# scraed/LanPaint

Measured on AMD Instinct MI355X. Metric: langevin_think_iterations_per_sec, higher is better.
Workload: dtype f32; 1 GPU; c2_sdxl: latent 1x4x128x128 per GPU, 30 sigmas x 5 think iterations, 50% box mask, stub backbone x->(0.9x,0.8x), VE/Karras schedule; rng=torch, graph=auto, mask_format=f32, mask_seen_by_kernels=bits, captured_calls=1, backbone_io=f32, replicas=1, rows_per_gpu=1, global_rows=1, latent_elements_per_gpu=65536

## Files before the change

### __graft_entry__.py

```python
from __future__ import annotations

import os
import subprocess
import sys

ROOT = os.path.dirname(os.path.abspath(__file__))
if ROOT not in sys.path:
    sys.path.insert(0, ROOT)


def build() -> None:
    from lanpaint_amd import build as lp_build
    lp_build.build(force=False, verbose=True)
    subprocess.run(["make", "-s", "-C", os.path.join(ROOT, "oracle")], check=True)
    import lanpaint_amd
    from lanpaint_amd import _cabi
    lib = _cabi.load()
    assert lib.lp_abi_version() == _cabi.ABI_VERSION
    print("lanpaint_amd", lanpaint_amd.__version__, "->", _cabi.LIB_PATH)


def smoke() -> None:
    import numpy as np
    import torch
    from lanpaint_amd import LanPaint
    from oracle.lanpaint_oracle import OracleLanPaint, times_from_sigma
    from tests.stubs import LinearTupleModel

    assert torch.cuda.is_available(), "smoke() needs a HIP device"
    dev = torch.device("cuda", 0)
    rng = np.random.default_rng(0)
    shape = (1, 4, 16, 16)
    y = rng.standard_normal(shape, dtype=np.float32)
    noise = rng.standard_normal(shape, dtype=np.float32)
    sigma = np.float32([1.5])
    x = (y + noise * sigma[0]).astype(np.float32)
    mask = np.zeros(shape, dtype=np.float32)
    mask[..., :8] = 1.0
    times = times_from_sigma(sigma, False)
    draws = [rng.standard_normal(shape, dtype=np.float32) for _ in range(5)]

    it = iter(draws)
# ... 42 lines not shown
```

### lanpaint_amd/build.py

```python
from __future__ import annotations

import os
import shutil
import subprocess
import sys

HERE = os.path.dirname(os.path.abspath(__file__))
ROOT = os.path.dirname(HERE)
CSRC = os.path.join(HERE, "csrc")
SOURCES = ["step_kernel.hip", "aux_kernels.hip", "blend_kernel.hip", "videomask_kernel.hip", "audio_kernel.hip",
           "detail_kernel.hip", "label_kernel.hip", "color_kernel.hip", "fill_kernel.hip",
           "multiband_kernel.hip", "refine_kernel.hip", "stabilize_kernel.hip", "grain_kernel.hip",
           "propagate_kernel.hip", "temporal_fill_kernel.hip", "temporal_smooth_kernel.hip",
           "shot_kernel.hip", "cabi.hip"]
HEADERS = [os.path.join(CSRC, "lp_common.h"), os.path.join(CSRC, "mask_tile.h"), os.path.join(CSRC, "resample_tile.h"),
           os.path.join(CSRC, "motion_tile.h"), os.path.join(CSRC, "exports.map"), os.path.join(ROOT, "include", "lanpaint_hip.h")]
OUT = os.path.join(HERE, "liblanpaint_hip.so")


def _hipcc():
    for cand in (os.environ.get("HIPCC"), shutil.which("hipcc"), "/opt/rocm/bin/hipcc"):
        if cand and os.path.exists(cand):
            return cand
    raise RuntimeError("hipcc not found (set HIPCC or install ROCm)")


def needs_build(out=OUT):
    if not os.path.exists(out):
        return True
    t = os.path.getmtime(out)
    deps = [os.path.join(CSRC, s) for s in SOURCES] + HEADERS
    return any(os.path.getmtime(p) > t for p in deps)


def build(force=False, verbose=True, shader_clock=False, trace=False):
    if trace:
        out = os.path.join(ROOT, "build", "liblanpaint_hip_trace.so")
        os.makedirs(os.path.dirname(out), exist_ok=True)
        return _compile(out, ["-DLP_TRACE_INSTANTIATIONS"], verbose) if force or needs_build(out) else out
    if shader_clock:
        out = os.path.join(ROOT, "build", "liblanpaint_hip_clk.so")
        os.makedirs(os.path.dirname(out), exist_ok=True)
        return _compile(out, ["-DLP_SHADER_CLOCK"], verbose) if force or needs_build(out) else out
    if not force and not needs_build():
        return OUT
    return _compile(OUT, [], verbose)


def _compile(out, extra, verbose):
    cmd = [_hipcc(), "--offload-arch=gfx950", "-O3", "-std=c++17", "-ffp-contract=on", "-fno-fast-math",
           "-fhip-fp32-correctly-rounded-divide-sqrt", "-fPIC", "-shared", "-fvisibility=hidden",
           "-Wl,--version-script=" + os.path.join(CSRC, "exports.map"),
           "-mllvm", "-amdgpu-kernarg-preload-count=14",
           "-I" + os.path.join(ROOT, "include"), "-I" + CSRC]
    cmd += extra + [os.path.join(CSRC, s) for s in SOURCES] + ["-o", out]
    if verbose:
        print(" ".join(cmd), flush=True)
    subprocess.run(cmd, check=True)
    return out


if __name__ == "__main__":
    build(force="--force" in sys.argv, shader_clock="--shader-clock" in sys.argv, trace="--trace" in sys.argv)
```

### lanpaint_amd/capture.py

```python
from __future__ import annotations

import ctypes
import os
import weakref

import torch

from . import _cabi
from ._util import _gc_hold, _gc_release
from .buffers import _CapturedCall, _Workspace
from .masks import _compact_mask


class GraphReplay:

    MAX_GRAPHS = 16
    AUTO_MAX_BACKBONE_HOST_US = 100.0

    def begin_call(self, x, latent_image, noise, sigma, latent_mask, current_times, model_options, seed):
        cap = self._last_cap
        if cap is None or cap.tail is None or self.model_dtype is not None or not x.is_cuda:
            return None
        self.img_dim_size = len(x.shape)
        self.latent_image, self.noise = latent_image, noise
        self.audio_indicator = self.current_times_audio = self.audio_correction = None
        self._noise_regenerated = self._noise_is_zero(noise)
        if not self._same_call(cap, x, sigma, latent_mask, current_times, cap.ident[4], model_options, seed):
            return None
        lib, stream = self._lib, self._stream(x.device)
        ve, abt = current_times[0], current_times[1]
        out = torch.empty_like(x)
        k0 = cap.k0_desc
# ... 45 lines not shown
        if table is None or table[3] != len(self._graphs) or table[4] is not model_options:
            nd.valid_word = self._rng_state(x.device).data_ptr() + 32
            table = self._node_table(cap0, nd.n_steps, model_options, nd)
        stream = self._stream(x.device)
        ve, abt = current_times[0], current_times[1]
        out = torch.empty_like(x)
        k0 = cap0.k0_desc
        k0.x, k0.noise = x.data_ptr(), noise.data_ptr()
        k0.t_ve, k0.t_abt, k0.t_rsig = ve.data_ptr(), abt.data_ptr(), sigma.data_ptr()
        k0.t_model = (current_times[2] if cap0.flow else ve).data_ptr()
        k0.io_table_val[0], k0.io_table_val[1] = k0.x, out.data_ptr()
        off = 0
        if self.rng == "torch":
            gen = self._generator(x.device)
            off = gen.get_offset()
            k0.rng_state_val[0], k0.rng_state_val[1] = off, gen.initial_seed()
        if getattr(nd, "_lp_table", None) is not table:
            nd._lp_table = table
            nd.replace, nd.exec_by_count, nd.n_counts = table[2], table[0], len(table[1])
            nd.valid_word = self._rng_state(x.device).data_ptr() + 32
            nd.full_exec_by_count, nd.full_binding_by_count = table[5], table[6]
        rc = self._lib.lp_node_call(ctypes.byref(nd), stream)
        if rc != _cabi.LP_OK:
            try:
                self._rng_state(x.device)[4] = 1
            except Exception:
                pass
            self._forget_captures()
            _cabi.check(rc, "lp_node_call")
        n_eff = nd.n_eff
        if not nd.launched:
            cap0.node_table = None
            return self(x, latent_image, noise, sigma, latent_mask, current_times, model_options, seed, n_steps=n_eff), n_eff
        cap = table[1][n_eff]
        if self.rng == "torch" and cap.launches:
            self._generator(x.device).set_offset(off + cap.launches)
            self._torch_consumed += cap.launches
        self._iterations_run += cap.ran
        self.last_inner_steps = cap.ran
        return out, n_eff

    def _forget_captures(self):
        self._last_cap = None
        for cap in self._graphs.values():
            cap.alive = False
            cap.node_table = None
            cap.siblings = {}
        self._graphs.clear()

    def _node_table(self, cap0, n_max, model_options, nd=None):
        caps = []
        for n in range(int(n_max) + 1):
            cap = cap0 if cap0.ident[4] == n else cap0.siblings.get(n)
            if cap is None or not cap.alive:
                cap = self._graphs.get(cap0.key[:2] + (n,) + cap0.key[3:])
                if cap is not None and (cap.tail is None or cap.model_options is not model_options or cap.ws is not cap0.ws):
                    cap = None
                if cap is not None:
                    cap0.siblings[n] = cap
            caps.append(cap if (cap is not None and cap.tail is not None) else None)
        arr = (ctypes.c_void_p * len(caps))(*[(c.tail.graph_exec if c is not None else None) for c in caps])
        full = full_b = None
        if nd is not None and os.environ.get("LANPAINT_AMD_NODE_ONE_LAUNCH", "1") != "0":
# ... 407 lines not shown
```

### lanpaint_amd/csrc/cabi.hip

```cpp
#include <cmath>

#include "lp_common.h"

namespace lp {
int step_dispatch(const lp_step_desc* d, hipStream_t stream, void* timer);
int replace_node_update(const lp_step_desc* d, hipGraphExec_t exec, const lp_graph_binding* b);
int timer_create(void** out);
int timer_destroy(void* h);
int timer_elapsed_ns(void* h, double* ns);
int coeffs_dispatch(const lp_hyper* h, const float* ve, int ve_stride, const float* abt, int abt_stride,
                    const float* rs, int rs_stride, const float* step_ov, int step_stride, const float* t_model,
                    int t_stride, int rows, float* table, hipStream_t stream);
int finalize_dispatch(const lp_final_desc* d, hipStream_t stream);
int sigma_times_dispatch(const float* sigma, int rows, const float* schedule, int schedule_len, int is_flow, float* times,
                         float* scalars, int32_t* seq_out, int32_t seq, hipStream_t stream);
int sigma_times_rule_dispatch(const float* sigma, int rows, const float* schedule, int schedule_len, int is_flow,
                              float* times, float* scalars, int32_t* seq_out, int32_t seq, int32_t n_steps, int32_t early_stop,
                              int32_t total_steps, double min_step_frac, int32_t guess, uint64_t* valid_out, hipStream_t stream);
int blend_dispatch(const lp_blend_desc* d, hipStream_t stream);
int philox_dispatch(float* out, int64_t n_el, uint64_t seed, uint64_t offset, uint32_t slot, hipStream_t stream);
int ring_dispatch(const float* mask, float* ring, int64_t planes, int height, int width, hipStream_t stream);
int wmse_dispatch(const float* a, const float* b, const float* mask, const float* ring, int64_t n_el, double* acc,
                  double* scratch, int scratch_blocks, hipStream_t stream);
int torch_normal_dispatch(float* out, int64_t n, uint64_t seed, uint64_t offset, uint32_t bg, hipStream_t stream);
// ... 400 lines not shown
int lp_graph_release(void* tail_graph, void* tail_exec) {
    if (tail_exec) (void)hipGraphExecDestroy(static_cast<hipGraphExec_t>(tail_exec));
    if (tail_graph) (void)hipGraphDestroy(static_cast<hipGraph_t>(tail_graph));
    return LP_OK;
}

int32_t lp_effective_inner_steps(int32_t n_steps, double step_f, double frac, int32_t total_steps, int32_t early_stop,
                                 double min_step_frac) {
    return lp::effective_inner_steps(n_steps, step_f, frac, total_steps, early_stop, min_step_frac);
}

static int node_wait(const lp_node_call_desc* c, int32_t want, hipStream_t s) {
    for (int32_t k = 0; k < c->spin_limit; ++k)
        if (__atomic_load_n(c->seq_out, __ATOMIC_ACQUIRE) == want) return LP_OK;
    if (hipStreamSynchronize(s) != hipSuccess) return LP_E_LAUNCH;
    return __atomic_load_n(c->seq_out, __ATOMIC_ACQUIRE) == want ? LP_OK : LP_E_LAUNCH;
}

static int node_call_body(lp_node_call_desc* c, hipStream_t s, bool* queued_spec) {
    const auto exec_for = [&](int32_t n) -> hipGraphExec_t {
        return (c->exec_by_count && n >= 0 && n < c->n_counts) ? static_cast<hipGraphExec_t>(c->exec_by_count[n]) : nullptr;
    };
    const bool speculate = c->guess >= 0 && c->valid_word && exec_for(c->guess) != nullptr && c->replace && !c->replace->es_reset;
    c->speculated = speculate ? 1 : 0;
    c->hit = 0;
    c->launched = 0;
    int rc = LP_OK;
    lp_step_desc rep;
    if (c->replace) {
        rep = *c->replace;
        rep.io_valid = 0;
    }
    lp_step_desc d;
    bool fold_sigma = speculate && c->fold_sigma && c->is_flow == ((c->replace->flags & LP_FL_FLOW) ? 1 : 0) &&
                      c->rows == c->replace->rows;
    if (fold_sigma) {
        d = rep;
        d.phases |= LP_PH_SIGMA;
        d.sg_sigma = c->sigma; d.sg_schedule = c->schedule; d.sg_schedule_len = c->schedule_len; d.sg_times_out = c->times_out;
        d.sg_scalars_out = c->scalars_out; d.sg_seq_out = c->seq_out; d.sg_seq = c->seq; d.sg_valid_out = c->valid_word;
        d.sg_n_steps = c->n_steps; d.sg_early_stop = c->early_stop; d.sg_total_steps = c->total_steps; d.sg_guess = c->guess;
        d.sg_min_step_frac = c->min_step_frac;
        lp::StepPlan plan;
        fold_sigma = lp::plan_step(d, &plan) == LP_OK;
    }
    c->one_launch = 0;
    if (fold_sigma) {
        hipGraphExec_t full = (c->full_exec_by_count && c->full_binding_by_count && c->guess < c->n_counts)
                                  ? static_cast<hipGraphExec_t>(c->full_exec_by_count[c->guess]) : nullptr;
        const lp_graph_binding* fb = full ? c->full_binding_by_count[c->guess] : nullptr;
        if (full && fb) {
            rc = lp::replace_node_update(&d, full, fb);
            if (rc != LP_OK) return rc;
            if (hipGraphLaunch(full, s) != hipSuccess) return LP_E_LAUNCH;
            *queued_spec = true;
            c->one_launch = 1;
        } else {
            rc = lp::step_dispatch(&d, s, nullptr);
            if (rc != LP_OK) return rc;
            *queued_spec = true;
        }
    } else {
        rc = lp::sigma_times_rule_dispatch(c->sigma, c->rows, c->schedule, c->schedule_len, c->is_flow, c->times_out,
                                           c->scalars_out, c->seq_out, c->seq, c->n_steps, c->early_stop, c->total_steps,
                                           c->min_step_frac, speculate ? c->guess : -1, c->valid_word, s);
        if (rc != LP_OK) return rc;
        *queued_spec = speculate;
        if (c->replace) {
            rc = lp::step_dispatch(&rep, s, nullptr);
            if (rc != LP_OK) return rc;
        }
    }
    if (speculate && !c->one_launch && hipGraphLaunch(exec_for(c->guess), s) != hipSuccess) return LP_E_LAUNCH;
    rc = node_wait(c, c->seq, s);
    if (rc != LP_OK) return rc;
    c->step_f = c->scalars_out[0];
    c->frac = c->scalars_out[1];
    c->n_eff = lp::effective_inner_steps(c->n_steps, static_cast<double>(c->step_f), static_cast<double>(c->frac),
                                         c->total_steps, c->early_stop, c->min_step_frac);
    if (c->valid_word && static_cast<int32_t>(c->scalars_out[3]) != c->n_eff) return LP_E_UNSUPPORTED;
    if (speculate) {
        if (c->n_eff == c->guess) {
            c->hit = 1;
            c->launched = 1;
// ... 84 lines not shown
```

### lanpaint_amd/csrc/lp_common.h

```cpp
#pragma once
#include <hip/hip_runtime.h>
#include <hip/hip_ext.h>
#include <stdint.h>

#include "lanpaint_hip.h"

namespace lp {

constexpr int kWave = 64;

__device__ __forceinline__ int nearest_exact_index(int i, int in_size, int out_size, int rule) {
#pragma clang fp contract(off)
    const float scale = static_cast<float>(in_size) / static_cast<float>(out_size);
    const float at = static_cast<float>(i) + 0.5f;
    int s;
    if (rule == LP_NN_ATEN_SCALAR) {
        s = static_cast<int>(floorf(at * scale));
    } else {
        float src = (rule == LP_NN_ATEN_CPU_GENERIC_FMA) ? __builtin_fmaf(scale, at, -0.5f) : (scale * at - 0.5f);
        src = src < 0.0f ? 0.0f : src;
        s = static_cast<int>(floorf(static_cast<float>(static_cast<double>(src) + 0.5)));
    }
    return s < in_size - 1 ? s : in_size - 1;
}
// ... 583 lines not shown
}

struct StepPlan {
    const void* kernel;
    dim3 grid;
    uint32_t ph_ct;
    int vec;
    bool decide;
    int decide_slot;
    int mode, x0w, rng, es;
    bool st;
};
struct StepArgs {
    void* x_t;
    void* C;
    const void *a2, *a3, *a4, *a5;
    int32_t el_per_row;
    uint32_t flags;
    void* ptr[9];
};
int plan_step(const lp_step_desc& d, StepPlan* out, bool timed = false);
void pack_step_args(const StepPlan& p, const lp_step_desc& d, StepArgs* a);
bool plan_is_node(const StepPlan& p, const void* func, const dim3& grid, const dim3& block);

__device__ __forceinline__ int code_of(float v) {
    const float t = v > 0.0f ? (v < 1.0f ? v : 1.0f) : 0.0f;
    return static_cast<int>(__fadd_rn(__fmul_rn(t, 255.0f), 0.5f));
}

__device__ __forceinline__ double capped_distance(int32_t q) {
    const uint32_t mag = q < 0 ? 0u - static_cast<uint32_t>(q) : static_cast<uint32_t>(q);
    const double r = sqrt(static_cast<double>(mag < 4096u ? mag : 4096u));
    return q < 0 ? -r : r;
}

}
```

### lanpaint_amd/csrc/step_kernel.hip

```cpp
#include <cstddef>

#include "lp_common.h"

#pragma clang fp contract(off)

namespace lp {

struct RegionCoef {
    float e_full, k_full, std_full, e_half, k_half, std_half, dt, a, cx0, cxt;
};

struct RowCoef {
    float scale, sqrt_abt, oma, abt, rsigma, dtx, dty, ax, ay, dx, dy, valid;
    RegionCoef reg[2];
    float rscale;
};

__device__ __forceinline__ RowCoef load_row(const float* __restrict__ coef, int row) {
    const float* c = coef + static_cast<int64_t>(row) * LP_COEF_STRIDE;
    RowCoef r;
    r.scale = c[LP_C_SCALE]; r.sqrt_abt = c[LP_C_SQRT_ABT]; r.oma = c[LP_C_OMA]; r.abt = c[LP_C_ABT];
    r.rsigma = c[LP_C_RSIGMA]; r.dtx = c[LP_C_DTX]; r.dty = c[LP_C_DTY]; r.ax = c[LP_C_AX]; r.ay = c[LP_C_AY];
    r.dx = c[LP_C_DX]; r.dy = c[LP_C_DY]; r.valid = c[LP_C_VALID];
    r.rscale = c[LP_C_RSCALE];
// ... 1482 lines not shown
static int enqueue(const StepPlan& p, const lp_step_desc& d, hipStream_t stream, Timer* timer) {
    LP_TRACE(p);
    StepArgs a;
    pack_step_args(p, d, &a);
    if (timer) (void)hipExtLaunchKernel(p.kernel, p.grid, dim3(kBlock), a.ptr, 0, stream, timer->start, timer->stop, 0);
    else (void)hipLaunchKernel(p.kernel, p.grid, dim3(kBlock), a.ptr, 0, stream);
    if (hipGetLastError() != hipSuccess) return LP_E_LAUNCH;
    if (p.decide) {
        hipLaunchKernelGGL(lp_es_decide_kernel, dim3(1), dim3(kWave), 0, stream, d, p.decide_slot);
        if (hipGetLastError() != hipSuccess) return LP_E_LAUNCH;
    }
    return LP_OK;
}

int step_dispatch(const lp_step_desc* dp, hipStream_t stream, void* timer_handle) {
    if (!dp) return LP_E_INVALID;
    Timer* timer = static_cast<Timer*>(timer_handle);
    StepPlan p;
    const int rc = plan_step(*dp, &p, timer != nullptr);
    return rc == LP_OK ? enqueue(p, *dp, stream, timer) : rc;
}

int replace_node_update(const lp_step_desc* dp, hipGraphExec_t exec, const lp_graph_binding* b) {
    if (!dp || !exec || !b || !b->node || !b->func) return LP_E_INVALID;
    const lp_step_desc& d = *dp;
    if (!(d.phases & LP_PH_REPLACE) || d.xi_post || d.xi_pre || (d.flags & LP_FL_X0S_GIVEN)) return LP_E_INVALID;
    StepPlan p;
    const int rc = plan_step(d, &p);
    if (rc != LP_OK) return rc;
    if (!plan_is_node(p, b->func, dim3(b->grid[0], b->grid[1], b->grid[2]), dim3(b->block[0], b->block[1], b->block[2])))
        return LP_E_INVALID;
    StepArgs a;
    pack_step_args(p, d, &a);
    hipKernelNodeParams np{};
    np.func = const_cast<void*>(p.kernel);
    np.gridDim = p.grid;
    np.blockDim = dim3(kBlock);
    np.sharedMemBytes = b->shared_bytes;
    np.kernelParams = a.ptr;
    np.extra = nullptr;
    return hipGraphExecKernelNodeSetParams(exec, static_cast<hipGraphNode_t>(b->node), &np) == hipSuccess ? LP_OK : LP_E_LAUNCH;
}

int timer_create(void** out) {
    if (!out) return LP_E_INVALID;
    Timer* t = new Timer();
    if (hipEventCreate(&t->start) != hipSuccess || hipEventCreate(&t->stop) != hipSuccess) {
        delete t;
        return LP_E_LAUNCH;
    }
    *out = t;
    return LP_OK;
// ... 23 lines not shown
```

### lanpaint_amd/nodes.py

```python
from __future__ import annotations

import math
import os
import weakref
from contextlib import contextmanager

import torch

from . import _cabi, interp_rule
from .blend import MaskBlend, gaussian_kernel_2d, merge_video_with_mask
from .image_nodes import LanPaint_ImageDecode, LanPaint_ImageEncode, _snap_mask_nearest_exact
from .resample import _hip_device, _resample
from .lanpaint import LanPaint, pack_mask, raw_stream, refresh_packed_mask, tensor_version
from .types import FusedCFGHeads

try:
    import comfy
    import comfy.samplers
    from comfy.model_base import ModelType
    HAVE_COMFY = True
except Exception:
    comfy = None
    HAVE_COMFY = False

    class ModelType:
        FLUX = "FLUX"
        FLOW = "FLOW"
        FLOW_AV = "FLOW_AV"

try:
    import comfyui_version
    _ver = tuple(int(p) if p.isdigit() else 0 for p in comfyui_version.__version__.split("."))
# ... 162 lines not shown
                                          self.conds.get("positive", None), self.cfg, self.cfg_BIG,
                                          model_options=model_options, seed=seed)


class KSamplerX0Inpaint:

    def __init__(self, model, sigmas):
        self.inner_model = model
        self.sigmas = sigmas
        self.audio_indicator = None
        self.audio_shifts = None
        self._mask_cache = None
        self._mailbox = None
        self._seq = 0
        self._node_desc = None
        self._node_static = None
        self._speculate = os.environ.get("LANPAINT_AMD_SPECULATE", "1") != "0"
        self._last_step = None
        self._spec_misses = 0
        self._spec_hist = []
        self._n_eff_table = None
        self._sched = None
        self._times = None

    def _guess_inner_steps(self, nd, rows, flow):
        if self._last_step is None or self._spec_misses >= 2 or not self._speculate:
            return -1
        tab = self._n_eff_table
        key = (rows, flow, nd.n_steps, nd.early_stop, nd.min_step_frac)
        if tab is None or tab[0] != key:
            import numpy as np
            sched = self._sched[1].detach().cpu().numpy().astype(np.float32)
            one = np.float32(1.0)
            counts = []
            for j, s in enumerate(sched):
                if flow:
                    a = one - s
                    abt = (a * a) / (a * a + s * s) if (a * a + s * s) != 0 else np.float32(np.nan)
                else:
                    abt = one / (one + s * s)
                acc = np.float32(0.0)
                for _ in range(rows):
                    acc = np.float32(acc + np.float32(one - abt))
                frac = float(np.float32(acc / np.float32(rows)))
                counts.append(-1 if frac != frac else
                              _cabi.load().lp_effective_inner_steps(nd.n_steps, float(j), frac, nd.total_steps, nd.early_stop,
                                                                    nd.min_step_frac))
            self._n_eff_table = tab = (key, counts)
        j = self._last_step + 1
        return tab[1][j] if 0 <= j < len(tab[1]) else -1

    def _mailbox_views(self):
        if self._mailbox is None:
            mb = torch.zeros(4, dtype=torch.float32).pin_memory()
            self._mailbox = (mb, mb.numpy(), mb.view(torch.int32).numpy())
        return self._mailbox

    def _wait_mailbox(self, seq, device):
        _mb, f32, i32 = self._mailbox
        for _ in range(20000):
            if i32[2] == seq:
                break
        else:
            torch.cuda.current_stream(device).synchronize()
            if i32[2] != seq:
                raise RuntimeError("lp_sigma_times mailbox was not written (sequence %d, found %d)" % (seq, int(i32[2])))
        return float(f32[0]), float(f32[1])

    def _latent_mask(self, denoise_mask):
        c = self._mask_cache
        ver = (tensor_version(denoise_mask), denoise_mask.data_ptr())
        if (c is not None and c[0]() is denoise_mask and c[1][1] == ver[1] and denoise_mask.is_cuda
                and (c[1][0] != ver[0] or ver[0] == -1) and getattr(c[2], "_lp_bits", None) is not None):
            refresh_packed_mask(c[2], denoise_mask)
            self._mask_cache = c = (c[0], ver, c[2])
            return c[2]
        if c is None or c[0]() is not denoise_mask or c[1] != ver:
            if denoise_mask.is_cuda:
                latent_mask = pack_mask(denoise_mask, denoise_mask=True)
            else:
                latent_mask = 1 - (denoise_mask > 0.5).float()
            self._mask_cache = c = (weakref.ref(denoise_mask), ver, latent_mask)
        return c[2]

    def __call__(self, x, sigma, denoise_mask, model_options={}, seed=None, **kwargs):
        model_type = self.inner_model.inner_model.model_type
        IS_FLUX = model_type == ModelType.FLUX
        IS_FLOW = model_type in FLOW_MODEL_TYPES
        fused_seq = None
        if (sigma.is_cuda and sigma.dtype == torch.float32 and sigma.ndim == 1 and self.sigmas.is_cuda
                and self.sigmas.dtype == torch.float32 and self.sigmas.device == sigma.device):
            sc = self._sched
            if sc is None or sc[0] is not self.sigmas:
                dense = self.sigmas.contiguous()
                self._sched = sc = (self.sigmas, dense, dense.data_ptr(), dense.numel(), len(self.sigmas) - 1)
            sig_c = sigma if sigma.is_contiguous() else sigma.contiguous()
            rows = sig_c.shape[0]
            tm = self._times
            if tm is None or tm[0] != rows or tm[1] != sigma.device:
                sets = []
                for _ in range(2):
                    b = torch.empty((3 * rows,), dtype=torch.float32, device=sigma.device)
                    sets.append((b[:rows], b[rows:2 * rows], b[2 * rows:3 * rows], b))
                self._times = tm = (rows, sigma.device, sets)
            VE_Sigma, abt, Flow_t, buf = tm[2][self._seq & 1]
            mb = self._mailbox_views()[0]
            self._seq = fused_seq = (self._seq % 0x7ffffff0) + 1
            pm = getattr(self, "PaintMethod", None)
            if (denoise_mask is not None and self.audio_indicator is None and "denoise_mask_function" not in model_options
                    and getattr(pm, "_last_cap", None) is not None and sigma.device.index == torch.cuda.current_device()
                    and type(self.LanPaint_early_stop) is int and type(pm.n_steps) is int):
                nd = self._node_desc
                if nd is None:
                    nd = self._node_desc = _cabi.LpNodeCallDesc()
                    nd.spin_limit = 200000
                    nd.fold_sigma = int(os.environ.get("LANPAINT_AMD_FOLD_SIGMA", "1") != "0")
                static = (rows, sc[2], sc[3], bool(IS_FLUX or IS_FLOW), pm.n_steps, self.LanPaint_early_stop, sc[4],
                          getattr(self, "LanPaint_min_step_frac", 1.0), mb)
                if self._node_static != static:
                    self._node_static = static
                    nd.rows, nd.schedule, nd.schedule_len, nd.is_flow = rows, sc[2], sc[3], int(static[3])
                    nd.scalars_out, nd.seq_out = mb.data_ptr(), mb.data_ptr() + 8
                    nd.n_steps, nd.early_stop, nd.total_steps = int(pm.n_steps), int(self.LanPaint_early_stop), sc[4]
                    nd.min_step_frac = float(static[7])
                nd.sigma, nd.seq, nd.times_out = sig_c.data_ptr(), fused_seq, buf.data_ptr()
                nd.guess = self._guess_inner_steps(nd, rows, static[3])
                res = pm.node_call(x, self.latent_image, self.noise, sigma, self._latent_mask(denoise_mask),
                                   (VE_Sigma, abt, Flow_t), model_options, seed, nd)
                if res is not None:
                    out = res[0]
                    self._last_step = int(nd.step_f)
                    if nd.speculated:
                        self._spec_hist = (self._spec_hist + [bool(nd.hit)])[-4:]
                        if self._spec_hist.count(False) >= 2:
                            self._spec_misses = 2
                    step_i = model_options.get("i", kwargs.get("i", 0))
                    if step_i % 2 == 0:
                        cb = model_options.get("callback", None)
                        if cb is not None:
                            cb({"i": step_i, "denoised": out, "x": x})
                    return out
            args = (sig_c.data_ptr(), rows, sc[2], sc[3], int(bool(IS_FLUX or IS_FLOW)), buf.data_ptr(),
                    mb.data_ptr(), mb.data_ptr() + 8, fused_seq, raw_stream(sigma.device))
            if sigma.device.index == torch.cuda.current_device():
                _cabi.check(_cabi.load().lp_sigma_times_mailbox(*args), "lp_sigma_times_mailbox")
            else:
                with torch.cuda.device(sigma.device):
                    _cabi.check(_cabi.load().lp_sigma_times_mailbox(*args), "lp_sigma_times_mailbox")
        elif IS_FLUX or IS_FLOW:
            Flow_t = sigma
            abt = (1 - Flow_t) ** 2 / ((1 - Flow_t) ** 2 + Flow_t ** 2)
            VE_Sigma = Flow_t / (1 - Flow_t)
        else:
            VE_Sigma = sigma
            abt = 1 / (1 + VE_Sigma ** 2)
            Flow_t = (1 - abt) ** 0.5 / ((1 - abt) ** 0.5 + abt ** 0.5)

        current_times_audio = audio_correction = None
        if self.audio_indicator is not None and self.audio_shifts is not None and time_shift_sigma is not None:
            shift_v, shift_a = self.audio_shifts
            Flow_a = time_shift_sigma(Flow_t, shift_v, shift_a)
            abt_a = (1 - Flow_a) ** 2 / ((1 - Flow_a) ** 2 + Flow_a ** 2)
            current_times_audio = (Flow_a / (1 - Flow_a), abt_a, Flow_a)
# ... 387 lines not shown
```

Before: 125,500 think-iterations/s.

## Add native C++ node-call fast path that replays captured graphs without Python

Adds a pybind/torch C++ extension (NodeFast) that snapshots the engine state after a successful captured node call. On later calls it validates a list of watched attributes, tensor pins and versions natively, then calls lp_node_call directly, skipping the Python sampler-facing path. The native node call also reorders descriptor setup so a planned graph update reuses the already computed step plan. This targets per-call host overhead in a workload dominated by small kernels. In exchange it adds a large snapshot/validation surface where stale-state bugs are possible, plus a build dependency that falls back to Python if missing.

```diff
diff --git a/__graft_entry__.py b/__graft_entry__.py
--- a/__graft_entry__.py
+++ b/__graft_entry__.py
@@ -18,6 +18,8 @@
     lib = _cabi.load()
     assert lib.lp_abi_version() == _cabi.ABI_VERSION
     print("lanpaint_amd", lanpaint_amd.__version__, "->", _cabi.LIB_PATH)
+    from lanpaint_amd import nodefast
+    print("native node-call entry:", getattr(nodefast.load(), "__file__", "not built (the Python path is the path)"))
 
 
 def smoke() -> None:
diff --git a/lanpaint_amd/build.py b/lanpaint_amd/build.py
--- a/lanpaint_amd/build.py
+++ b/lanpaint_amd/build.py
@@ -16,6 +16,8 @@
 HEADERS = [os.path.join(CSRC, "lp_common.h"), os.path.join(CSRC, "mask_tile.h"), os.path.join(CSRC, "resample_tile.h"),
            os.path.join(CSRC, "motion_tile.h"), os.path.join(CSRC, "exports.map"), os.path.join(ROOT, "include", "lanpaint_hip.h")]
 OUT = os.path.join(HERE, "liblanpaint_hip.so")
+NODE_FAST_SOURCE = "node_fast.cpp"
+NODE_FAST_OUT = os.path.join(HERE, "_node_fast.so")
 
 
 def _hipcc():
@@ -42,9 +44,40 @@
         out = os.path.join(ROOT, "build", "liblanpaint_hip_clk.so")
         os.makedirs(os.path.dirname(out), exist_ok=True)
         return _compile(out, ["-DLP_SHADER_CLOCK"], verbose) if force or needs_build(out) else out
-    if not force and not needs_build():
-        return OUT
-    return _compile(OUT, [], verbose)
+    out = OUT if (not force and not needs_build()) else _compile(OUT, [], verbose)
+    build_node_fast(force=force, verbose=verbose)
+    return out
+
+
+def build_node_fast(force=False, verbose=True):
+    src, hdr = os.path.join(CSRC, NODE_FAST_SOURCE), os.path.join(ROOT, "include", "lanpaint_hip.h")
+    if not force and os.path.exists(NODE_FAST_OUT) and os.path.getmtime(NODE_FAST_OUT) >= max(os.path.getmtime(src), os.path.getmtime(hdr)):
+        return NODE_FAST_OUT
+    try:
+        import sysconfig
+        import pybind11
+        import torch
+        from torch.utils import cpp_extension
+        cxx = os.environ.get("CXX") or shutil.which("g++") or shutil.which("c++") or shutil.which("clang++")
+        if cxx is None:
+            raise RuntimeError("no C++ compiler found (set CXX)")
+        rocm = os.environ.get("ROCM_PATH") or os.path.dirname(os.path.dirname(os.path.realpath(_hipcc())))
+        incs = cpp_extension.include_paths() + [pybind11.get_include(), sysconfig.get_paths()["include"],
+                                                os.path.join(rocm, "include"), os.path.join(ROOT, "include")]
+        libdir = os.path.join(os.path.dirname(torch.__file__), "lib")
+        cmd = [cxx, "-O2", "-std=c++17", "-fPIC", "-shared", "-fvisibility=hidden", "-D__HIP_PLATFORM_AMD__=1", "-DUSE_ROCM=1",
+               "-D_GLIBCXX_USE_CXX11_ABI=%d" % int(torch._C._GLIBCXX_USE_CXX11_ABI)]
+        cmd += ["-I" + p for p in incs] + [src, "-o", NODE_FAST_OUT, "-L" + libdir, "-Wl,-rpath," + libdir,
+                                           "-lc10", "-lc10_hip", "-ltorch_cpu", "-ltorch", "-ltorch_python"]
+        if verbose:
+            print(" ".join(cmd), flush=True)
+        subprocess.run(cmd, check=True)
+        return NODE_FAST_OUT
+    except Exception as e:
+        import warnings
+        warnings.warn("lanpaint_amd: the native node-call entry was not built (%s: %s); the sampler-facing path stays in Python"
+                      % (type(e).__name__, str(e).splitlines()[0] if str(e) else ""))
+        return None
 
 
 def _compile(out, extra, verbose):
diff --git a/lanpaint_amd/capture.py b/lanpaint_amd/capture.py
--- a/lanpaint_amd/capture.py
+++ b/lanpaint_amd/capture.py
@@ -7,7 +7,7 @@
 import torch
 
 from . import _cabi
-from ._util import _gc_hold, _gc_release
+from ._util import _gc_hold, _gc_release, tensor_version
 from .buffers import _CapturedCall, _Workspace
 from .masks import _compact_mask
 
@@ -99,16 +99,10 @@
             nd.full_exec_by_count, nd.full_binding_by_count = table[5], table[6]
         rc = self._lib.lp_node_call(ctypes.byref(nd), stream)
         if rc != _cabi.LP_OK:
-            try:
-                self._rng_state(x.device)[4] = 1
-            except Exception:
-                pass
-            self._forget_captures()
-            _cabi.check(rc, "lp_node_call")
+            self._node_call_failed(rc, x.device)
         n_eff = nd.n_eff
         if not nd.launched:
-            cap0.node_table = None
-            return self(x, latent_image, noise, sigma, latent_mask, current_times, model_options, seed, n_steps=n_eff), n_eff
+            return self._node_call_uncaptured(x, sigma, latent_mask, current_times, model_options, seed, n_eff), n_eff
         cap = table[1][n_eff]
         if self.rng == "torch" and cap.launches:
             self._generator(x.device).set_offset(off + cap.launches)
@@ -116,6 +110,47 @@
         self._iterations_run += cap.ran
         self.last_inner_steps = cap.ran
         return out, n_eff
+
+    def _node_call_failed(self, rc, dev):
+        try:
+            self._rng_state(dev)[4] = 1
+        except Exception:
+            pass
+        self._forget_captures()
+        _cabi.check(rc, "lp_node_call")
+
+    def _node_call_uncaptured(self, x, sigma, latent_mask, current_times, model_options, seed, n_eff):
+        if self._last_cap is not None:
+            self._last_cap.node_table = None
+        return self(x, self.latent_image, self.noise, sigma, latent_mask, current_times, model_options, seed, n_steps=n_eff)
+
+    def node_fast_state(self, x, sigma, latent_mask, current_times, model_options, seed, nd):
+        cap0 = self._last_cap
+        table = None if cap0 is None else cap0.node_table
+        if (table is None or getattr(nd, "_lp_table", None) is not table or table[3] != len(self._graphs)
+                or table[4] is not model_options or self.rng not in ("torch", "philox") or not isinstance(model_options, dict)
+                or not self._same_call(cap0, x, sigma, latent_mask, current_times, cap0.ident[4], model_options, seed)
+                or (tensor_version(self.noise) == -1 and not self.assume_static_noise)):
+            return None
+        t, own = type(self), ("langevin_dynamics", "score_model", "prepare_step_size", "node_call")
+        if any(n in self.__dict__ for n in own) or not isinstance(self._lib.lp_node_call, ctypes._CFuncPtr):
+            return None
+        ident = lambda o, *names: [(o, n, getattr(o, n, None), False) for n in names]
+        value = lambda o, *names: [(o, n, getattr(o, n), True) for n in names]
+        watches = (ident(self, "_last_cap", "latent_image", "noise", "audio_indicator", "audio_correction", "_noise_regenerated",
+                         "_noise_check", "assume_static_noise", "rng", "graph", "model_dtype", "__class__", "__dict__", "_lib")
+                   + value(self, "img_dim_size", "n_steps", "chara_lamb", "chara_beta", "step_size", "min_step_frac",
+                           "early_stop_threshold", "early_stop_patience", "IS_FLUX", "IS_FLOW")
+                   + ident(t, *own) + ident(cap0, "node_table", "tail", "ident", "k0_desc")
+                   + ident(latent_mask, "_lp_bits", "_lp_u8") + ident(nd, "_lp_table"))
+        caps = table[1]
+        return {"engine": self, "watches": watches, "absent": [(self.__dict__, n) for n in own],
+                "options_absent": ["lanpaint_semantic_stop"], "graphs": self._graphs, "n_graphs": len(self._graphs),
+                "replace_desc": ctypes.addressof(cap0.k0_desc), "flow_times": bool(cap0.flow), "rng_torch": self.rng == "torch",
+                "generator": self._generator(x.device) if self.rng == "torch" else None,
+                "launches": [int(c.launches) if c is not None else 0 for c in caps],
+                "ran": [int(c.ran) if c is not None else 0 for c in caps],
+                "node_call": ctypes.cast(self._lib.lp_node_call, ctypes.c_void_p).value, "keep": (table, cap0, nd)}
 
     def _forget_captures(self):
         self._last_cap = None
diff --git a/lanpaint_amd/csrc/cabi.hip b/lanpaint_amd/csrc/cabi.hip
--- a/lanpaint_amd/csrc/cabi.hip
+++ b/lanpaint_amd/csrc/cabi.hip
@@ -446,44 +446,54 @@
         return (c->exec_by_count && n >= 0 && n < c->n_counts) ? static_cast<hipGraphExec_t>(c->exec_by_count[n]) : nullptr;
     };
     const bool speculate = c->guess >= 0 && c->valid_word && exec_for(c->guess) != nullptr && c->replace && !c->replace->es_reset;
-    c->speculated = speculate ? 1 : 0;
-    c->hit = 0;
-    c->launched = 0;
     int rc = LP_OK;
-    lp_step_desc rep;
-    if (c->replace) {
-        rep = *c->replace;
-        rep.io_valid = 0;
-    }
     lp_step_desc d;
+    lp::StepPlan plan;
     bool fold_sigma = speculate && c->fold_sigma && c->is_flow == ((c->replace->flags & LP_FL_FLOW) ? 1 : 0) &&
                       c->rows == c->replace->rows;
     if (fold_sigma) {
-        d = rep;
+        d = *c->replace;
+        d.io_valid = 0;
         d.phases |= LP_PH_SIGMA;
         d.sg_sigma = c->sigma; d.sg_schedule = c->schedule; d.sg_schedule_len = c->schedule_len; d.sg_times_out = c->times_out;
         d.sg_scalars_out = c->scalars_out; d.sg_seq_out = c->seq_out; d.sg_seq = c->seq; d.sg_valid_out = c->valid_word;
         d.sg_n_steps = c->n_steps; d.sg_early_stop = c->early_stop; d.sg_total_steps = c->total_steps; d.sg_guess = c->guess;
         d.sg_min_step_frac = c->min_step_frac;
-        lp::StepPlan plan;
         fold_sigma = lp::plan_step(d, &plan) == LP_OK;
     }
-    c->one_launch = 0;
+    const auto publish = [&](int32_t one) {
+        c->speculated = speculate ? 1 : 0;
+        c->hit = 0;
+        c->launched = 0;
+        c->one_launch = one;
+    };
+    int32_t one_launch = 0;
     if (fold_sigma) {
         hipGraphExec_t full = (c->full_exec_by_count && c->full_binding_by_count && c->guess < c->n_counts)
                                   ? static_cast<hipGraphExec_t>(c->full_exec_by_count[c->guess]) : nullptr;
         const lp_graph_binding* fb = full ? c->full_binding_by_count[c->guess] : nullptr;
         if (full && fb) {
-            rc = lp::replace_node_update(&d, full, fb);
-            if (rc != LP_OK) return rc;
-            if (hipGraphLaunch(full, s) != hipSuccess) return LP_E_LAUNCH;
+            rc = lp::replace_node_update_planned(plan, d, full, fb);
+            if (rc == LP_OK && hipGraphLaunch(full, s) != hipSuccess) rc = LP_E_LAUNCH;
+            if (rc != LP_OK) {
+                publish(0);
+                return rc;
+            }
             *queued_spec = true;
-            c->one_launch = 1;
-        } else {
-            rc = lp::step_dispatch(&d, s, nullptr);
-            if (rc != LP_OK) return rc;
-            *queued_spec = true;
+            one_launch = 1;
         }
+    }
+    publish(one_launch);
+    lp_step_desc rep;
+    if (c->replace) {
+        rep = *c->replace;
+        rep.io_valid = 0;
+    }
+    if (one_launch) {
+    } else if (fold_sigma) {
+        rc = lp::step_dispatch(&d, s, nullptr);
+        if (rc != LP_OK) return rc;
+        *queued_spec = true;
     } else {
         rc = lp::sigma_times_rule_dispatch(c->sigma, c->rows, c->schedule, c->schedule_len, c->is_flow, c->times_out,
                                            c->scalars_out, c->seq_out, c->seq, c->n_steps, c->early_stop, c->total_steps,
diff --git a/lanpaint_amd/csrc/lp_common.h b/lanpaint_amd/csrc/lp_common.h
--- a/lanpaint_amd/csrc/lp_common.h
+++ b/lanpaint_amd/csrc/lp_common.h
@@ -629,6 +629,7 @@
 int plan_step(const lp_step_desc& d, StepPlan* out, bool timed = false);
 void pack_step_args(const StepPlan& p, const lp_step_desc& d, StepArgs* a);
 bool plan_is_node(const StepPlan& p, const void* func, const dim3& grid, const dim3& block);
+int replace_node_update_planned(const StepPlan& p, const lp_step_desc& d, hipGraphExec_t exec, const lp_graph_binding* b);
 
 __device__ __forceinline__ int code_of(float v) {
     const float t = v > 0.0f ? (v < 1.0f ? v : 1.0f) : 0.0f;
diff --git a/lanpaint_amd/csrc/node_fast.cpp b/lanpaint_amd/csrc/node_fast.cpp
--- /dev/null
+++ b/lanpaint_amd/csrc/node_fast.cpp
@@ -0,0 +1,294 @@
+#include <torch/extension.h>
+#include <torch/csrc/autograd/python_variable.h>
+#include <c10/hip/HIPFunctions.h>
+#include <c10/hip/HIPStream.h>
+
+#include <chrono>
+#include <cstdint>
+#include <mutex>
+#include <string>
+#include <vector>
+
+#include "lanpaint_hip.h"
+
+namespace py = pybind11;
+
+namespace {
+
+using node_call_fn = int (*)(lp_node_call_desc*, void*);
+
+struct Watch {
+    py::object obj, name, expect;
+    bool eq;
+};
+
+struct TensorPin {
+    at::Tensor t;
+    const void* ptr = nullptr;
+    int64_t version = -1;
+};
+
+int64_t version_of(const at::Tensor& t) { return t.is_inference() ? -1 : static_cast<int64_t>(t._version()); }
+
+bool pin_ok(const TensorPin& p) { return p.t.data_ptr() == p.ptr && version_of(p.t) == p.version; }
+
+TensorPin pin(const py::handle& h) {
+    if (!THPVariable_Check(h.ptr())) throw py::type_error("NodeFast: expected a tensor");
+    TensorPin p;
+    p.t = THPVariable_Unpack(h.ptr());
+    p.ptr = p.t.data_ptr();
+    p.version = version_of(p.t);
+    return p;
+}
+
+bool dense_f32(const at::Tensor& t) { return t.scalar_type() == at::kFloat && t.is_contiguous(); }
+
+class NodeFast {
+public:
+    explicit NodeFast(const py::dict& c) {
+        owner_ = c["owner"];
+        engine_ = c["engine"];
+        for (const py::handle& h : c["watches"]) {
+            const py::tuple w = py::reinterpret_borrow<py::tuple>(h);
+            watches_.push_back({py::reinterpret_borrow<py::object>(w[0]), py::reinterpret_borrow<py::object>(w[1]),
+                                py::reinterpret_borrow<py::object>(w[2]), w[3].cast<bool>()});
+        }
+        for (const py::handle& h : c["absent"]) {
+            const py::tuple w = py::reinterpret_borrow<py::tuple>(h);
+            if (!PyDict_Check(w[0].ptr())) throw py::type_error("NodeFast: 'absent' wants (dict, key)");
+            absent_.emplace_back(py::reinterpret_borrow<py::object>(w[0]), py::reinterpret_borrow<py::object>(w[1]));
+        }
+        model_options_ = c["model_options"];
+        if (!PyDict_Check(model_options_.ptr())) throw py::type_error("NodeFast: model_options must be a dict");
+        for (const py::handle& h : c["options_absent"]) options_absent_.push_back(py::reinterpret_borrow<py::object>(h));
+        seed_ = c["seed"];
+        graphs_ = c["graphs"];
+        n_graphs_ = c["n_graphs"].cast<Py_ssize_t>();
+        denoise_mask_obj_ = c["denoise_mask"];
+        denoise_mask_ = pin(denoise_mask_obj_);
+        latent_mask_obj_ = c["latent_mask"];
+        latent_mask_ = pin(latent_mask_obj_);
+        refresh_ = c["refresh_mask"];
+        latent_image_ = pin(c["latent_image"]);
+        noise_ = pin(c["noise"]);
+        for (const py::handle& h : c["time_bufs"]) time_bufs_.push_back(pin(h));
+        if (time_bufs_.size() != 2) throw py::value_error("NodeFast: two time buffers");
+        rows_ = c["rows"].cast<int64_t>();
+        sigma_numel_ = c["sigma_numel"].cast<int64_t>();
+        for (const TensorPin& b : time_bufs_)
+            if (b.t.numel() != 3 * rows_ || !dense_f32(b.t)) throw py::value_error("NodeFast: time buffer is not fp32 [3 * rows]");
+        shape_ = c["shape"].cast<std::vector<int64_t>>();
+        const at::Tensor x = THPVariable_Unpack(c["x"].ptr());
+        device_ = x.device();
+        flow_times_ = c["flow_times"].cast<bool>();
+        nd_ = reinterpret_cast<lp_node_call_desc*>(c["node_desc"].cast<uintptr_t>());
+        k0_ = reinterpret_cast<lp_step_desc*>(c["replace_desc"].cast<uintptr_t>());
+        fn_ = reinterpret_cast<node_call_fn>(c["node_call"].cast<uintptr_t>());
+        if (!nd_ || !k0_ || !fn_) throw py::value_error("NodeFast: null descriptor or entry");
+        rng_torch_ = c["rng_torch"].cast<bool>();
+        if (rng_torch_) generator_ = c["generator"].cast<at::Generator>();
+        guess_by_step_ = c["guess_by_step"].cast<std::vector<int32_t>>();
+        launches_ = c["launches"].cast<std::vector<int64_t>>();
+        ran_ = c["ran"].cast<std::vector<int64_t>>();
+        if (launches_.size() != ran_.size() || static_cast<int64_t>(launches_.size()) != nd_->n_counts)
+            throw py::value_error("NodeFast: per-count tables do not fit the descriptor");
+        keep_ = c["keep"];
+        for (const char* n : {"_seq", "_last_step", "_spec_misses", "_spec_hist", "_torch_consumed", "_iterations_run", "last_inner_steps"})
+            names_.push_back(py::reinterpret_steal<py::object>(PyUnicode_InternFromString(n)));
+    }
+
+    py::object call(const py::handle& x_h, const py::handle& sigma_h, const py::handle& mask_h, const py::handle& options,
+                    const py::handle& seed) {
+        const py::object none = py::none();
+        t_entry_ = now_ns();
+        if (mask_h.ptr() != denoise_mask_obj_.ptr() || options.ptr() != model_options_.ptr()) return none;
+        if (!THPVariable_Check(x_h.ptr()) || !THPVariable_Check(sigma_h.ptr())) return none;
+        if (seed.ptr() != seed_.ptr()) {
+            if (Py_TYPE(seed.ptr()) != Py_TYPE(seed_.ptr())) return none;
+            const int same = PyObject_RichCompareBool(seed.ptr(), seed_.ptr(), Py_EQ);
+            if (same != 1) { PyErr_Clear(); return none; }
+        }
+        for (const Watch& w : watches_) {
+            PyObject* v = PyObject_GetAttr(w.obj.ptr(), w.name.ptr());
+            if (!v) { PyErr_Clear(); v = Py_None; Py_INCREF(v); }
+            bool ok = v == w.expect.ptr();
+            if (!ok && w.eq && Py_TYPE(v) == Py_TYPE(w.expect.ptr())) {
+                const int same = PyObject_RichCompareBool(v, w.expect.ptr(), Py_EQ);
+                if (same < 0) PyErr_Clear();
+                ok = same == 1;
+            }
+            Py_DECREF(v);
+            if (!ok) return none;
+        }
+        for (const auto& a : absent_)
+            if (PyDict_Contains(a.first.ptr(), a.second.ptr()) != 0) { PyErr_Clear(); return none; }
+        for (const py::object& k : options_absent_)
+            if (PyDict_Contains(options.ptr(), k.ptr()) != 0) { PyErr_Clear(); return none; }
+        if (PyObject_Length(graphs_.ptr()) != n_graphs_) { PyErr_Clear(); return none; }
+
+        const at::Tensor& x = THPVariable_Unpack(x_h.ptr());
+        const at::Tensor& sigma = THPVariable_Unpack(sigma_h.ptr());
+        if (x.device() != device_ || sigma.device() != device_ || !dense_f32(x) || !dense_f32(sigma) || sigma.dim() != 1 ||
+            sigma.size(0) != rows_ || sigma.numel() != sigma_numel_ || !x.sizes().equals(shape_) ||
+            (reinterpret_cast<uintptr_t>(x.data_ptr()) & 15) != 0)
+            return none;
+        if (!pin_ok(denoise_mask_) || !pin_ok(latent_mask_) || !pin_ok(latent_image_) || !pin_ok(noise_) ||
+            !pin_ok(time_bufs_[0]) || !pin_ok(time_bufs_[1]))
+            return none;
+        const at::Tensor& nz = noise_.t;
+        if (!dense_f32(nz) || !nz.sizes().equals(shape_) || (reinterpret_cast<uintptr_t>(nz.data_ptr()) & 15) != 0) return none;
+        void* stream = nullptr;
+        if (device_.is_cuda()) {
+            if (c10::hip::current_device() != device_.index()) return none;
+            stream = c10::hip::getCurrentHIPStream(device_.index()).stream();
+        }
+
+        long seq = 0, last_step = -1, spec_misses = 0;
+        if (!read_long(owner_, 0, &seq, nullptr) || !read_long(owner_, 2, &spec_misses, nullptr)) return none;
+        bool no_step = false;
+        if (!read_long(owner_, 1, &last_step, &no_step)) return none;
+        const int set = static_cast<int>(seq & 1);
+        const int32_t new_seq = static_cast<int32_t>(seq % 0x7ffffff0) + 1;
+        int32_t guess = -1;
+        if (!no_step && spec_misses < 2 && last_step + 1 >= 0 && last_step + 1 < static_cast<long>(guess_by_step_.size()))
+            guess = guess_by_step_[static_cast<size_t>(last_step + 1)];
+
+        if (!refresh_.is_none()) refresh_(latent_mask_obj_, denoise_mask_obj_);
+        at::Tensor out = at::empty_like(x);
+        uint64_t off = 0;
+        float* const tb = static_cast<float*>(time_bufs_[set].t.data_ptr());
+        k0_->x = static_cast<const float*>(x.data_ptr());
+        k0_->noise = static_cast<const float*>(nz.data_ptr());
+        k0_->t_ve = tb;
+        k0_->t_abt = tb + rows_;
+        k0_->t_rsig = static_cast<const float*>(sigma.data_ptr());
+        k0_->t_model = flow_times_ ? tb + 2 * rows_ : tb;
+        k0_->io_table_val[0] = reinterpret_cast<uint64_t>(x.data_ptr());
+        k0_->io_table_val[1] = reinterpret_cast<uint64_t>(out.data_ptr());
+        if (rng_torch_) {
+            std::lock_guard<std::mutex> lock(generator_.mutex());
+            off = generator_.get_offset();
+            k0_->rng_state_val[0] = off;
+            k0_->rng_state_val[1] = generator_.current_seed();
+        }
+        nd_->sigma = static_cast<const float*>(sigma.data_ptr());
+        nd_->seq = new_seq;
+        nd_->times_out = tb;
+        nd_->guess = guess;
+        if (!write_long(owner_, 0, new_seq)) throw py::error_already_set();
+        int rc;
+        {
+            py::gil_scoped_release release;
+            t_launch_ = now_ns();
+            rc = fn_(nd_, stream);
+            t_back_ = now_ns();
+        }
+        if (rc != LP_OK) return py::int_(rc);
+        const int32_t n_eff = nd_->n_eff;
+        if (!nd_->launched || n_eff < 0 || n_eff >= static_cast<int32_t>(launches_.size())) return py::make_tuple(none, n_eff, set);
+        const int64_t draws = launches_[static_cast<size_t>(n_eff)], ran = ran_[static_cast<size_t>(n_eff)];
+        if (rng_torch_ && draws) {
+            {
+                std::lock_guard<std::mutex> lock(generator_.mutex());
+                generator_.set_offset(off + static_cast<uint64_t>(draws));
+            }
+            if (!add_long(engine_, 4, draws)) throw py::error_already_set();
+        }
+        if (!add_long(engine_, 5, ran) || !write_long(engine_, 6, ran) ||
+            !write_long(owner_, 1, static_cast<long>(nd_->step_f)))
+            throw py::error_already_set();
+        if (nd_->speculated) note_guess(nd_->hit != 0);
+        return py::make_tuple(py::reinterpret_steal<py::object>(THPVariable_Wrap(out)), n_eff);
+    }
+
+    py::tuple last_ns() const { return py::make_tuple(t_entry_, t_launch_, t_back_); }
+
+private:
+    static int64_t now_ns() {
+        return std::chrono::duration_cast<std::chrono::nanoseconds>(std::chrono::steady_clock::now().time_since_epoch()).count();
+    }
+
+    bool read_long(const py::object& o, int name, long* v, bool* is_none) {
+        PyObject* a = PyObject_GetAttr(o.ptr(), names_[name].ptr());
+        if (!a) { PyErr_Clear(); return false; }
+        bool ok = true;
+        if (a == Py_None && is_none) {
+            *is_none = true;
+        } else if (PyLong_CheckExact(a)) {
+            *v = PyLong_AsLong(a);
+            if (*v == -1 && PyErr_Occurred()) { PyErr_Clear(); ok = false; }
+        } else {
+            ok = false;
+        }
+        Py_DECREF(a);
+        return ok;
+    }
+
+    bool write_long(const py::object& o, int name, long v) {
+        PyObject* a = PyLong_FromLong(v);
+        if (!a) return false;
+        const int rc = PyObject_SetAttr(o.ptr(), names_[name].ptr(), a);
+        Py_DECREF(a);
+        return rc == 0;
+    }
+
+    bool add_long(const py::object& o, int name, int64_t d) {
+        PyObject* a = PyObject_GetAttr(o.ptr(), names_[name].ptr());
+        if (!a) return false;
+        PyObject* b = PyLong_FromLongLong(d);
+        PyObject* s = b ? PyNumber_Add(a, b) : nullptr;
+        Py_DECREF(a);
+        Py_XDECREF(b);
+        if (!s) return false;
+        const int rc = PyObject_SetAttr(o.ptr(), names_[name].ptr(), s);
+        Py_DECREF(s);
+        return rc == 0;
+    }
+
+    void note_guess(bool hit) {
+        py::list hist;
+        PyObject* old = PyObject_GetAttr(owner_.ptr(), names_[3].ptr());
+        if (!old) throw py::error_already_set();
+        const py::object held = py::reinterpret_steal<py::object>(old);
+        for (const py::handle& h : held) hist.append(h);
+        hist.append(py::bool_(hit));
+        while (py::len(hist) > 4) PySequence_DelItem(hist.ptr(), 0);
+        int misses = 0;
+        for (const py::handle& h : hist) misses += h.ptr() == Py_False ? 1 : 0;
+        if (PyObject_SetAttr(owner_.ptr(), names_[3].ptr(), hist.ptr()) != 0) throw py::error_already_set();
+        if (misses >= 2 && !write_long(owner_, 2, 2)) throw py::error_already_set();
+    }
+
+    py::object owner_, engine_, model_options_, seed_, graphs_, denoise_mask_obj_, latent_mask_obj_, refresh_, keep_;
+    std::vector<Watch> watches_;
+    std::vector<std::pair<py::object, py::object>> absent_;
+    std::vector<py::object> options_absent_, names_;
+    Py_ssize_t n_graphs_ = 0;
+    TensorPin denoise_mask_, latent_mask_, latent_image_, noise_;
+    std::vector<TensorPin> time_bufs_;
+    int64_t rows_ = 0, sigma_numel_ = 0;
+    std::vector<int64_t> shape_;
+    c10::Device device_{c10::kCPU};
+    bool flow_times_ = false, rng_torch_ = false;
+    lp_node_call_desc* nd_ = nullptr;
+    lp_step_desc* k0_ = nullptr;
+    node_call_fn fn_ = nullptr;
+    int64_t t_entry_ = 0, t_launch_ = 0, t_back_ = 0;
+    at::Generator generator_;
+    std::vector<int32_t> guess_by_step_;
+    std::vector<int64_t> launches_, ran_;
+};
+
+}
+
+PYBIND11_MODULE(_node_fast, m) {
+    m.doc() = "native steady-state entry of the sampler-facing sigma call (see lanpaint_amd/nodes.py)";
+    m.attr("ABI_VERSION") = LP_ABI_VERSION;
+    m.attr("NODE_DESC_BYTES") = sizeof(lp_node_call_desc);
+    m.attr("STEP_DESC_BYTES") = sizeof(lp_step_desc);
+    py::class_<NodeFast>(m, "NodeFast")
+        .def(py::init<const py::dict&>())
+        .def("call", &NodeFast::call)
+        .def("last_ns", &NodeFast::last_ns,
+             "(entry, before lp_node_call, after it) of the last call that was taken, on time.perf_counter_ns's clock");
+}
diff --git a/lanpaint_amd/csrc/step_kernel.hip b/lanpaint_amd/csrc/step_kernel.hip
--- a/lanpaint_amd/csrc/step_kernel.hip
+++ b/lanpaint_amd/csrc/step_kernel.hip
@@ -1528,12 +1528,15 @@
 }
 
 int replace_node_update(const lp_step_desc* dp, hipGraphExec_t exec, const lp_graph_binding* b) {
-    if (!dp || !exec || !b || !b->node || !b->func) return LP_E_INVALID;
-    const lp_step_desc& d = *dp;
+    if (!dp) return LP_E_INVALID;
+    StepPlan p;
+    const int rc = plan_step(*dp, &p);
+    return rc == LP_OK ? replace_node_update_planned(p, *dp, exec, b) : rc;
+}
+
+int replace_node_update_planned(const StepPlan& p, const lp_step_desc& d, hipGraphExec_t exec, const lp_graph_binding* b) {
+    if (!exec || !b || !b->node || !b->func) return LP_E_INVALID;
     if (!(d.phases & LP_PH_REPLACE) || d.xi_post || d.xi_pre || (d.flags & LP_FL_X0S_GIVEN)) return LP_E_INVALID;
-    StepPlan p;
-    const int rc = plan_step(d, &p);
-    if (rc != LP_OK) return rc;
     if (!plan_is_node(p, b->func, dim3(b->grid[0], b->grid[1], b->grid[2]), dim3(b->block[0], b->block[1], b->block[2])))
         return LP_E_INVALID;
     StepArgs a;
diff --git a/lanpaint_amd/nodefast.py b/lanpaint_amd/nodefast.py
--- /dev/null
+++ b/lanpaint_amd/nodefast.py
@@ -0,0 +1,58 @@
+from __future__ import annotations
+
+import ctypes
+import os
+import warnings
+
+from . import _cabi
+
+_mod = False
+
+
+def enabled() -> bool:
+    return os.environ.get("LANPAINT_AMD_NODE_FAST", "1") != "0"
+
+
+def snapshot(k, x, sigma, denoise_mask, latent_mask, current_times, model_options, seed, nd, rows, flow):
+    from ._util import tensor_version
+    from .lanpaint import refresh_packed_mask
+    pm = k.PaintMethod
+    if (k._fast_mod is None or k._fast_strikes >= 3 or not hasattr(pm, "node_fast_state")
+            or not hasattr(k, "LanPaint_min_step_frac")):
+        return None
+    cfg = pm.node_fast_state(x, sigma, latent_mask, current_times, model_options, seed, nd)
+    if cfg is None:
+        return None
+    base = k.inner_model.inner_model
+    ident = lambda o, *names: [(o, n, getattr(o, n, None), False) for n in names]
+    counts = list(k._inner_step_counts(nd, rows, flow)[1]) if k._speculate else []
+    cfg["watches"] = (ident(k, "inner_model", "sigmas", "_sched", "_times", "_mailbox", "_node_desc", "_node_static", "_mask_cache",
+                            "audio_indicator", "PaintMethod", "_speculate", "latent_image", "noise", "_fast_mod", "_n_eff_table")
+                      + ident(k.inner_model, "inner_model") + [(base, "model_type", base.model_type, True)]
+                      + [(k, n, getattr(k, n), True) for n in ("LanPaint_early_stop", "LanPaint_min_step_frac")]
+                      + cfg["watches"])
+    cfg["options_absent"] = cfg["options_absent"] + ["denoise_mask_function"]
+    stale_unseen = tensor_version(denoise_mask) == -1 and getattr(latent_mask, "_lp_bits", None) is not None
+    cfg.update(owner=k, model_options=model_options, seed=seed, x=x, shape=tuple(x.shape), rows=rows, sigma_numel=sigma.numel(),
+               denoise_mask=denoise_mask, latent_mask=latent_mask, refresh_mask=refresh_packed_mask if stale_unseen else None,
+               latent_image=k.latent_image, noise=k.noise, time_bufs=[s[3] for s in k._times[2]],
+               node_desc=ctypes.addressof(nd), guess_by_step=counts)
+    k._fast_served = 0
+    return k._fast_mod.NodeFast(cfg)
+
+
+def load():
+    global _mod
+    if _mod is False:
+        _mod = None
+        try:
+            import torch
+            from . import _node_fast as m
+            if (m.ABI_VERSION != _cabi.ABI_VERSION or m.STEP_DESC_BYTES != ctypes.sizeof(_cabi.LpStepDesc)
+                    or m.NODE_DESC_BYTES != ctypes.sizeof(_cabi.LpNodeCallDesc)):
+                raise ImportError("built against another lanpaint_hip.h (rebuild: python -m lanpaint_amd.build)")
+            _mod = m
+        except ImportError as e:
+            if os.path.exists(os.path.join(os.path.dirname(os.path.abspath(__file__)), "_node_fast.so")):
+                warnings.warn("lanpaint_amd: the native node-call entry does not load (%s); the sampler-facing path stays in Python" % e)
+    return _mod
diff --git a/lanpaint_amd/nodes.py b/lanpaint_amd/nodes.py
--- a/lanpaint_amd/nodes.py
+++ b/lanpaint_amd/nodes.py
@@ -7,7 +7,7 @@
 
 import torch
 
-from . import _cabi, interp_rule
+from . import _cabi, interp_rule, nodefast
 from .blend import MaskBlend, gaussian_kernel_2d, merge_video_with_mask
 from .image_nodes import LanPaint_ImageDecode, LanPaint_ImageEncode, _snap_mask_nearest_exact
 from .resample import _hip_device, _resample
@@ -216,10 +216,12 @@
         self._n_eff_table = None
         self._sched = None
         self._times = None
-
-    def _guess_inner_steps(self, nd, rows, flow):
-        if self._last_step is None or self._spec_misses >= 2 or not self._speculate:
-            return -1
+        self._fast = None
+        self._fast_mod = nodefast.load() if nodefast.enabled() else None
+        self._fast_served = 0
+        self._fast_strikes = 0
+
+    def _inner_step_counts(self, nd, rows, flow):
         tab = self._n_eff_table
         key = (rows, flow, nd.n_steps, nd.early_stop, nd.min_step_frac)
         if tab is None or tab[0] != key:
@@ -241,6 +243,12 @@
                               _cabi.load().lp_effective_inner_steps(nd.n_steps, float(j), frac, nd.total_steps, nd.early_stop,
                                                                     nd.min_step_frac))
             self._n_eff_table = tab = (key, counts)
+        return tab
+
+    def _guess_inner_steps(self, nd, rows, flow):
+        if self._last_step is None or self._spec_misses >= 2 or not self._speculate:
+            return -1
+        tab = self._inner_step_counts(nd, rows, flow)
         j = self._last_step + 1
         return tab[1][j] if 0 <= j < len(tab[1]) else -1
 
@@ -277,7 +285,39 @@
             self._mask_cache = c = (weakref.ref(denoise_mask), ver, latent_mask)
         return c[2]
 
+    def _after_node_call(self, out, nd, x, model_options, kwargs):
+        self._last_step = int(nd.step_f)
+        if nd.speculated:
+            self._spec_hist = (self._spec_hist + [bool(nd.hit)])[-4:]
+            if self._spec_hist.count(False) >= 2:
+                self._spec_misses = 2
+        return self._preview_hook(out, x, model_options, kwargs)
+
+    @staticmethod
+    def _preview_hook(out, x, model_options, kwargs):
+        step_i = model_options.get("i", kwargs.get("i", 0))
+        if step_i % 2 == 0:
+            cb = model_options.get("callback", None)
+            if cb is not None:
+                cb({"i": step_i, "denoised": out, "x": x})
+        return out
+
     def __call__(self, x, sigma, denoise_mask, model_options={}, seed=None, **kwargs):
+        fast = self._fast
+        if fast is not None:
+            res = fast.call(x, sigma, denoise_mask, model_options, seed)
+            if res is not None:
+                self._fast_served += 1
+                if type(res) is tuple and len(res) == 2:
+                    return self._preview_hook(res[0], x, model_options, kwargs)
+                self._fast = None
+                if type(res) is int:
+                    self.PaintMethod._node_call_failed(res, x.device)
+                times = self._times[2][res[2]][:3]
+                out = self.PaintMethod._node_call_uncaptured(x, sigma, self._mask_cache[2], times, model_options, seed, res[1])
+                return self._after_node_call(out, self._node_desc, x, model_options, kwargs)
+            self._fast = None
+            self._fast_strikes = 0 if self._fast_served else self._fast_strikes + 1
         model_type = self.inner_model.inner_model.model_type
         IS_FLUX = model_type == ModelType.FLUX
         IS_FLOW = model_type in FLOW_MODEL_TYPES
@@ -319,20 +359,14 @@
                     nd.min_step_frac = float(static[7])
                 nd.sigma, nd.seq, nd.times_out = sig_c.data_ptr(), fused_seq, buf.data_ptr()
                 nd.guess = self._guess_inner_steps(nd, rows, static[3])
-                res = pm.node_call(x, self.latent_image, self.noise, sigma, self._latent_mask(denoise_mask),
-                                   (VE_Sigma, abt, Flow_t), model_options, seed, nd)
+                latent_mask = self._latent_mask(denoise_mask)
+                res = pm.node_call(x, self.latent_image, self.noise, sigma, latent_mask, (VE_Sigma, abt, Flow_t),
+                                   model_options, seed, nd)
                 if res is not None:
-                    out = res[0]
-                    self._last_step = int(nd.step_f)
-                    if nd.speculated:
-                        self._spec_hist = (self._spec_hist + [bool(nd.hit)])[-4:]
-                        if self._spec_hist.count(False) >= 2:
-                            self._spec_misses = 2
-                    step_i = model_options.get("i", kwargs.get("i", 0))
-                    if step_i % 2 == 0:
-                        cb = model_options.get("callback", None)
-                        if cb is not None:
-                            cb({"i": step_i, "denoised": out, "x": x})
+                    out = self._after_node_call(res[0], nd, x, model_options, kwargs)
+                    if self._fast_mod is not None and nd.launched:
+                        self._fast = nodefast.snapshot(self, x, sigma, denoise_mask, latent_mask, (VE_Sigma, abt, Flow_t),
+                                                       model_options, seed, nd, rows, static[3])
                     return out
             args = (sig_c.data_ptr(), rows, sc[2], sc[3], int(bool(IS_FLUX or IS_FLOW)), buf.data_ptr(),
                     mb.data_ptr(), mb.data_ptr() + 8, fused_seq, raw_stream(sigma.device))
```

Result: no change. 125,100 think-iterations/s (-0.3%).
